# TrevorS/qwen3-tts-rs

Measured on AMD Instinct MI355X. Metric: acoustic_frames_per_sec, higher is better.
Workload: dtype bf16

## Files before the change

qwen3_tts_rs_amd/csrc/q3_codec_stream.hip:

```cpp
#include "q3_engine.h"

struct CsRow { int pos = 0; float* kv = nullptr; float* lat = nullptr; float* hist = nullptr; std::vector<float*> blocks; };
struct q3_codec_stream {
    q3_model* m = nullptr; int R = 0, cap = 0;
    int bf = 0, max_blocks = 0;
    std::vector<float*> free_blocks; int blocks_total = 0, blocks_in_use = 0, blocks_peak = 0;
    hipStream_t st = nullptr; bool owns_stream = false;
    std::vector<CsRow> rows;
    CodecWS ws;
    float *cs = nullptr, *sn = nullptr;
    char* desc = nullptr; size_t desc_cap = 0;
    float* stage = nullptr; float* stage_host = nullptr; size_t stage_cap = 0;
};

static size_t kv_floats(const q3_codec_stream* cs) {
    const q3_config& c = cs->m->cfg;
    return (size_t)c.dec_layers * 2 * c.dec_heads * c.dec_head_dim * cs->cap;
}

static size_t block_floats(const q3_codec_stream* cs) {
    const q3_config& c = cs->m->cfg;
    return ((size_t)c.dec_layers * 2 * c.dec_heads * c.dec_head_dim + c.dec_latent) * cs->bf;
}

q3_status codec_stream_create(q3_model* m, int rows, int max_frames, hipStream_t st, q3_codec_stream** out, int block_frames, int max_blocks) {
    if (!m || !m->finalized) return set_err(Q3_INVALID_ARG, "model not finalized");
    if (!out || rows < 1 || max_frames < 1) return set_err(Q3_INVALID_ARG, "q3_codec_stream_create: rows and max_frames must be positive");
    if (m->device < 0) return set_err(Q3_INVALID_ARG, "q3_codec_stream_create: the model has no device (manifest-only): the vocoder runs on the GPU");
    if (m->cfg.dec_head_dim != 64) return set_err(Q3_INVALID_ARG, "q3_codec_stream_create: decoder head dim must be 64");
    HIPC(hipSetDevice(m->device));
    std::unique_ptr<q3_codec_stream> cs(new q3_codec_stream());
    cs->m = m; cs->R = rows; cs->cap = max_frames; cs->rows.resize(rows);
    cs->bf = block_frames; cs->max_blocks = max_blocks;
    m->refs.fetch_add(1);
    auto fail = [&](q3_status s) { q3_codec_stream_free(cs.release()); return s; };
// ... 22 lines not shown
    if (max_blocks < 0) return set_err(Q3_INVALID_ARG, "q3_codec_stream_create_blocked: negative max_blocks");
    return codec_stream_create(m, rows, max_frames, nullptr, out, block_frames, max_blocks);
}
extern "C" q3_status q3_codec_stream_info(q3_codec_stream* cs, int* block_frames, size_t* block_bytes, int* blocks_total, int* blocks_in_use, int* blocks_peak) {
    if (!cs) return set_err(Q3_INVALID_ARG, "q3_codec_stream_info: null stream");
    if (block_frames) *block_frames = cs->bf;
    if (block_bytes) *block_bytes = block_floats(cs) * 4;
    if (blocks_total) *blocks_total = cs->blocks_total;
    if (blocks_in_use) *blocks_in_use = cs->blocks_in_use;
    if (blocks_peak) *blocks_peak = cs->blocks_peak;
    return Q3_OK;
}

extern "C" void q3_codec_stream_free(q3_codec_stream* cs) {
    if (!cs) return;
    q3_model* m = cs->m;
    (void)hipSetDevice(m->device);
    if (cs->st) (void)hipStreamSynchronize(cs->st);
    for (CsRow& r : cs->rows) { dev_free(r.kv); dev_free(r.lat); dev_free(r.hist); for (float* b : r.blocks) dev_free(b); }
    for (float* b : cs->free_blocks) dev_free(b);
    cs->ws.release();
    dev_free(cs->cs); dev_free(cs->sn); dev_free(cs->desc); dev_free(cs->stage);
    if (cs->stage_host) (void)hipHostFree(cs->stage_host);
    if (cs->owns_stream && cs->st) (void)hipStreamDestroy(cs->st);
    delete cs;
    if (m->refs.fetch_sub(1) == 1) model_destroy(m);
}

int codec_stream_pos(const q3_codec_stream* cs, int row) { return cs->rows[row].pos; }
void codec_stream_blocks(const q3_codec_stream* cs, int row, int upto, int* held, int* need) {
    const CsRow& r = cs->rows[row];
    *held = (int)r.blocks.size();
    *need = cs->bf ? std::max(0, (upto + cs->bf - 1) / cs->bf - *held) : 0;
}
void codec_stream_reset(q3_codec_stream* cs, int row) {
    CsRow& r = cs->rows[row];
    r.pos = 0;
    cs->blocks_in_use -= (int)r.blocks.size();
    cs->free_blocks.insert(cs->free_blocks.end(), r.blocks.begin(), r.blocks.end());
    r.blocks.clear();
}

extern "C" q3_status q3_codec_stream_reset(q3_codec_stream* cs, int row) {
    if (!cs || row < 0 || row >= cs->R) return set_err(Q3_INVALID_ARG, "q3_codec_stream_reset: bad row");
    codec_stream_reset(cs, row);
    return Q3_OK;
}
extern "C" q3_status q3_codec_stream_pos(q3_codec_stream* cs, int row, int* n_frames) {
    if (!cs || row < 0 || row >= cs->R || !n_frames) return set_err(Q3_INVALID_ARG, "q3_codec_stream_pos: bad row");
    *n_frames = cs->rows[row].pos;
    return Q3_OK;
}

namespace {
struct DescBlock {
    std::vector<char> host;
    template <typename T> size_t add(const std::vector<T>& v) {
        const size_t off = (host.size() + 15) & ~(size_t)15;
        host.resize(off + v.size() * sizeof(T));
        if (!v.empty()) memcpy(host.data() + off, v.data(), v.size() * sizeof(T));
        return off;
    }
};
}

q3_status codec_stream_push(q3_codec_stream* cs, const std::vector<CsPush>& all) {
    q3_model* m = cs->m;
    const q3_config& c = m->cfg;
    std::vector<CsPush> P;
    for (const CsPush& p : all) if (p.n > 0) P.push_back(p);
    q3_pcm_stage* ps = nullptr;
    std::vector<const CsPush*> flush;
    for (const CsPush& p : all) {
        if (p.ps) ps = p.ps;
        if (p.n_out) *p.n_out = 0;
        if (p.n <= 0 && p.ps && p.last) flush.push_back(&p);
    }
    if (P.empty()) {
        if (flush.empty()) return Q3_OK;
        std::vector<PsSeg> segs; std::vector<void*> outs; std::vector<size_t> cnt(flush.size(), 0);
        for (const CsPush* f : flush) { segs.push_back({f->ps_row, nullptr, 0, 1}); outs.push_back(f->out_host); }
        Q3C(pcm_stage_push_dev(ps, segs, cs->st, outs.data(), cnt.data()));
        for (size_t k = 0; k < flush.size(); ++k) if (flush[k]->n_out) *flush[k]->n_out = cnt[k];
        return Q3_OK;
    }
    HIPC(hipSetDevice(m->device));
    hipStream_t st = cs->st;
    const int Q = c.dec_q_dim, LAT = c.dec_latent, QD = c.dec_heads * c.dec_head_dim, cap = cs->cap, spf = samples_per_frame(c);
    const int nP = (int)P.size();
// ... 43 lines not shown
        CsRow& r = cs->rows[p.row];
        if (bf || r.kv) continue;
        if (dev_malloc((void**)&r.kv, kv_floats(cs) * 4) != hipSuccess || dev_malloc((void**)&r.lat, (size_t)LAT * cap * 4) != hipSuccess ||
            dev_malloc((void**)&r.hist, (size_t)Q * 2 * 4) != hipSuccess) {
            (void)hipGetLastError();
            dev_free(r.kv); dev_free(r.lat); dev_free(r.hist); r.kv = r.lat = r.hist = nullptr;
            return set_err(Q3_OOM, "codec stream: state of row %d (%zu MB)", p.row, (kv_floats(cs) + (size_t)LAT * cap) * 4 >> 20);
        }
    }
    int N = 0, W = 0, Lc = 0, solo_max = 0, max_tiles = 0;
    std::vector<int> col0(nP), out0(nP), conc, solo;
    for (int i = 0; i < nP; ++i) {
        const int f0 = cs->rows[P[i].row].pos, a0 = f0 + P[i].skip, e = f0 + P[i].n;
        col0[i] = N; N += P[i].n;
        out0[i] = W; W += e - a0;
        if (e > a0) {
            if (a0 > CODEC_CTX_FRAMES) { conc.push_back(i); Lc += e - a0 + CODEC_CTX_FRAMES; }
            else { solo.push_back(i); solo_max = std::max(solo_max, e); }
        }
        max_tiles = std::max(max_tiles, ((e - 1) >> 5) - (f0 >> 5) + 1);
    }
    const int Np = N + 2 * nP;
    {
        const int CS_WIDE = 2048;
        int max_n = 0; for (const CsPush& p : P) max_n = std::max(max_n, p.n);
        const int T = std::max(1, std::max(Lc, solo_max));
        const long long Tw = (long long)cs->R * (max_n + CODEC_CTX_FRAMES), Fw = (long long)cs->R * (max_n + 2);
        Q3C(codec_reserve(m, cs->ws, (int)std::max<long long>(T, std::min<long long>(Tw, CS_WIDE)),
                          (int)std::max<long long>(Np, std::min<long long>(Fw, CS_WIDE))));
    }
    CodecWS& ws = cs->ws;
    if ((size_t)W * spf > cs->stage_cap) {
        HIPC(hipStreamSynchronize(st));
        dev_free(cs->stage); cs->stage = nullptr;
        if (cs->stage_host) { (void)hipHostFree(cs->stage_host); cs->stage_host = nullptr; }
        cs->stage_cap = 0;
        HIPC(dev_malloc((void**)&cs->stage, (size_t)W * spf * 4));
        HIPC(hipHostMalloc((void**)&cs->stage_host, (size_t)W * spf * 4, hipHostMallocDefault));
        cs->stage_cap = (size_t)W * spf;
    }
    std::vector<PsSeg> psegs; std::vector<const CsPush*> pseg_of; std::vector<void*> pouts; PsPlan plan;
    if (ps) {
        for (int i = 0; i < nP; ++i)
            if (P[i].ps) { psegs.push_back({P[i].ps_row, cs->stage + (size_t)out0[i] * spf, (size_t)(P[i].n - P[i].skip) * spf, P[i].last}); pseg_of.push_back(&P[i]); }
        for (const CsPush* f : flush) { psegs.push_back({f->ps_row, nullptr, 0, 1}); pseg_of.push_back(f); }
        for (const CsPush* p : pseg_of) pouts.push_back(p->out_host);
        Q3C(pcm_stage_begin(ps, psegs, plan));
    }
    float *A = ws.bufA, *B = ws.bufB, *C = ws.bufC, *F = ws.bufF;
    float* knew = A + (size_t)QD * N;
    std::vector<int> pos(N);
    std::vector<AttnCsRow> arows(nP);
    std::vector<ColCopy> xin(Np), hist(2 * nP), compact(N), kvsc(N), latsc(N), latg(Lc), solog;
    std::vector<SegCopy> segs;
    std::vector<AttnCbRow> brows(bf ? nP : 0);
    std::vector<const float*> tabs;
    auto kv_col = [&](const CsRow& r, int f) { return bf ? r.blocks[f / bf] + f % bf : r.kv + f; };
    auto lat_col = [&](const CsRow& r, int f) { return bf ? r.blocks[f / bf] + lat_off + f % bf : r.lat + f; };
    std::vector<const uint32_t*> fsrc(on_dev ? N : 0);
    std::vector<uint32_t> fhost(on_dev ? 0 : (size_t)N * 16);
    for (int i = 0; i < nP; ++i) {
        const CsRow& r = cs->rows[P[i].row];
// ... 13 lines not shown
            else memcpy(&fhost[(size_t)col * 16], P[i].host + (size_t)j * 16, 64);
        }
    }
    {
        int l0 = 0;
        for (int i : conc) {
            const CsRow& r = cs->rows[P[i].row];
            const int a0 = r.pos + P[i].skip, c0 = a0 - CODEC_CTX_FRAMES, len = P[i].n - P[i].skip + CODEC_CTX_FRAMES;
            for (int j = 0; j < len; ++j) latg[l0 + j] = {lat_col(r, c0 + j), F + l0 + j, kp, Lc};
            segs.push_back({(unsigned long long)(l0 + CODEC_CTX_FRAMES) * spf, (unsigned long long)out0[i] * spf, (unsigned long long)(P[i].n - P[i].skip) * spf});
            l0 += len;
        }
        for (int i : solo) {
            const CsRow& r = cs->rows[P[i].row];
            const int e = r.pos + P[i].n;
            if (bf) for (int f = 0; f < e; ++f) solog.push_back({lat_col(r, f), F + f, kp, e});
            segs.push_back({(unsigned long long)(cs->rows[P[i].row].pos + P[i].skip) * spf, (unsigned long long)out0[i] * spf,
                            (unsigned long long)(P[i].n - P[i].skip) * spf});
        }
    }
    DescBlock db;
    const size_t o_pos = db.add(pos), o_arows = db.add(arows), o_xin = db.add(xin), o_hist = db.add(hist), o_compact = db.add(compact),
                 o_kvsc = db.add(kvsc), o_latsc = db.add(latsc), o_latg = db.add(latg), o_segs = db.add(segs), o_fsrc = db.add(fsrc),
                 o_brows = db.add(brows), o_tabs = db.add(tabs), o_solog = db.add(solog), o_ps = db.add(plan.desc);
    if (db.host.size() > cs->desc_cap) {
        HIPC(hipStreamSynchronize(st));
        dev_free(cs->desc); cs->desc = nullptr; cs->desc_cap = 0;
        HIPC(dev_malloc((void**)&cs->desc, db.host.size() * 2));
        cs->desc_cap = db.host.size() * 2;
    }
    struct Failed {
        q3_codec_stream* cs; const std::vector<CsPush>& P; bool armed = true;
        ~Failed() {
            if (!armed) return;
            (void)hipStreamSynchronize(cs->st);
            for (const CsPush& p : P) codec_stream_reset(cs, p.row);
        }
    } failed{cs, P};
    HIPC(q3_hipMemcpy(cs->desc, db.host.data(), db.host.size(), hipMemcpyHostToDevice));
    auto D = [&](size_t off) { return (const void*)(cs->desc + off); };
    if (on_dev) HIPC(launch_gather_frames((const uint32_t* const*)D(o_fsrc), ws.frames, N, st));
    else HIPC(q3_hipMemcpy(ws.frames, fhost.data(), fhost.size() * 4, hipMemcpyHostToDevice));

    const CodecScope scope(m);
    Q3C(codec_front_quant(m, ws, N, st));
    HIPC(launch_copy_cols((const ColCopy*)D(o_xin), Np, Q, 0, 0, st));
    HIPC(launch_copy_cols((const ColCopy*)D(o_hist), 2 * nP, Q, 0, 0, st));
    Q3C(codec_front_preconv(m, A, B, Np, st));
    HIPC(launch_copy_cols((const ColCopy*)D(o_compact), N, LAT, 0, 0, st));
    const float scale = (float)pow((double)c.dec_head_dim, -0.5);
    Q3C(codec_front_transformer(m, ws, N, st, [&](int l, float* q, float* k, float*, float* ao) -> q3_status {
        const size_t layer_off = (size_t)l * 2 * QD * kp;
        HIPC(launch_rope_c_pos(q, k, cs->cs, cs->sn, (const int*)D(o_pos), c.dec_heads, c.dec_head_dim, N, st));
        HIPC(launch_copy_cols((const ColCopy*)D(o_kvsc), N, 2 * QD, 0, layer_off, st));
        if (bf) HIPC(launch_attn_cb(q, ao, (const AttnCbRow*)D(o_brows), (const float* const*)D(o_tabs), nP, max_tiles, layer_off, c.dec_heads, c.dec_head_dim, N, bf, scale, st));
        else HIPC(launch_attn_cs(q, ao, (const AttnCsRow*)D(o_arows), nP, max_tiles, layer_off, c.dec_heads, c.dec_head_dim, N, cap, scale, st));
        return Q3_OK;
    }));
    HIPC(launch_copy_cols((const ColCopy*)D(o_latsc), N, LAT, 0, 0, st));
    const SegCopy* dsegs = (const SegCopy*)D(o_segs);
    if (!conc.empty()) {
        size_t max_n = 0; for (int i : conc) max_n = std::max(max_n, (size_t)(P[i].n - P[i].skip) * spf);
        HIPC(launch_copy_cols((const ColCopy*)D(o_latg), Lc, LAT, 0, 0, st));
        Q3C(codec_stack_dev(m, ws, F, Lc, st, nullptr, scope));
        HIPC(launch_copy_segs(ws.pcm, cs->stage, dsegs, (int)conc.size(), max_n, st));
    }
    for (size_t k = 0, g0 = 0; k < solo.size(); ++k) {
        const int i = solo[k]; const CsRow& r = cs->rows[P[i].row];
        const int e = r.pos + P[i].n;
        if (bf) { HIPC(launch_copy_cols((const ColCopy*)D(o_solog) + g0, e, LAT, 0, 0, st)); g0 += (size_t)e; }
        else HIPC(launch_copy_rows(r.lat, cap, F, e, LAT, e, st));
        Q3C(codec_stack_dev(m, ws, F, e, st, nullptr, scope));
        HIPC(launch_copy_segs(ws.pcm, cs->stage, dsegs + conc.size() + k, 1, (size_t)(P[i].n - P[i].skip) * spf, st));
    }
    bool raw = false;
    for (int i = 0; i < nP; ++i) raw = raw || !P[i].ps;
    if (W > 0 && raw) HIPC(hipMemcpyAsync(cs->stage_host, cs->stage, (size_t)W * spf * 4, hipMemcpyDeviceToHost, st));
    if (ps) Q3C(pcm_stage_run(ps, psegs, plan, (const PsDesc*)D(o_ps), st));
    HIPC(hipStreamSynchronize(st));
    if (ps) pcm_stage_finish(ps, psegs, plan, pouts.data(), nullptr);
    for (size_t k = 0; k < psegs.size(); ++k) if (pseg_of[k]->n_out) *pseg_of[k]->n_out = plan.count[k];
    for (int i = 0; i < nP; ++i) {
        if (P[i].pcm_host && !P[i].ps) memcpy(P[i].pcm_host, cs->stage_host + (size_t)out0[i] * spf, (size_t)(P[i].n - P[i].skip) * spf * 4);
        cs->rows[P[i].row].pos += P[i].n;
    }
    failed.armed = false; untake.armed = false;
    cs->blocks_peak = std::max(cs->blocks_peak, cs->blocks_in_use);
    return Q3_OK;
}

extern "C" q3_status q3_codec_stream_push(q3_codec_stream* cs, int n_rows, const int* rows, const uint32_t* const* frames_host,
                                          const int* n_frames, float* const* pcm_host, const size_t* cap) {
    if (!cs) return set_err(Q3_INVALID_ARG, "q3_codec_stream_push: null stream");
    if (n_rows < 0 || (n_rows > 0 && (!rows || !frames_host || !n_frames || !pcm_host || !cap)))
        return set_err(Q3_INVALID_ARG, "q3_codec_stream_push: null argument");
    const int spf = samples_per_frame(cs->m->cfg);
    std::vector<char> seen(cs->R, 0);
    std::vector<CsPush> P;
    for (int i = 0; i < n_rows; ++i) {
        const int r = rows[i], n = n_frames[i];
        if (r < 0 || r >= cs->R) return set_err(Q3_INVALID_ARG, "q3_codec_stream_push: row %d out of range (%d rows)", r, cs->R);
        if (seen[r]) return set_err(Q3_INVALID_ARG, "q3_codec_stream_push: row %d listed twice", r);
        seen[r] = 1;
        if (n < 0) return set_err(Q3_INVALID_ARG, "q3_codec_stream_push: negative frame count for row %d", r);
        if (n == 0) continue;
        if (cs->rows[r].pos + n > cs->cap)
// ... 61 lines not shown
```

qwen3_tts_rs_amd/csrc/q3_engine.h:

```cpp
#pragma once
#include "../../include/q3tts.h"
#include "q3_kernels.h"

#include <math.h>
#include <stdarg.h>
#include <stdio.h>
#include <string.h>

#include <algorithm>
#include <atomic>
#include <chrono>
#include <functional>
#include <memory>
#include <string>
#include <thread>
#include <mutex>
#include <unordered_map>
#include <vector>

#include "q3_internal.h"
#include "q3_aql.h"

using namespace q3;
#define Q3_HIDDEN __attribute__((visibility("hidden")))
// ... 317 lines not shown
    bool kv_bf16 = false, kv_in_bf16 = false; unsigned long long* kv_conv = nullptr;
    float *rows = nullptr, *embeds = nullptr, *xvec = nullptr; int n_rows_total = 0;
    uint32_t* ids_dev = nullptr; int *tr_dev = nullptr, *ci_dev = nullptr; float *proj_e = nullptr, *proj_h = nullptr;
    uint32_t* ref_codes_dev = nullptr;
    int *trail_base = nullptr, *trail_len = nullptr, *pad_row = nullptr;
    int* text_ready = nullptr;
    uint32_t* app_ids = nullptr; float *app_e = nullptr, *app_h = nullptr, *app_out = nullptr;
    int* flush_buf = nullptr; size_t flush_cap = 0;
    uint32_t* tok = nullptr; uint8_t* seen = nullptr; int *frame_idx = nullptr, *pos = nullptr, *token_count = nullptr;
    float* U = nullptr; uint32_t* codes = nullptr;
    float* logits_hist = nullptr; float* cp_logits_hist = nullptr; bool debug = false;
    bool prefilled = false; int frames_run = 0;
    uint64_t uid = 0; char* park_desc = nullptr; std::shared_ptr<ParkShelf> shelf;
    hipGraphExec_t graph_exec = nullptr; hipGraph_t graph = nullptr;
    q3::AqlProgram* aql = nullptr; int aql_mode = 0; bool aql_tried = false, aql_failed = false;
    bool precapture = false;
    CodecWS cws;
    q3_codec_stream* cstream = nullptr;
    q3_pcm_stage* ostage = nullptr; bool out_started = false;
    std::vector<OutSettings> out;
    hipStream_t dec_stream = nullptr; hipEvent_t dec_ev = nullptr;
    std::vector<CodecWS> par_ws; std::vector<hipStream_t> par_streams;
    CodecWS seg_ws;
    std::vector<uint32_t> codes_host; bool codes_host_valid = false;
    int stream_mode = 0;
    bool profile = false; ProfAcc prof_linear;
    bool legacy_attn = getenv("Q3_LEGACY_ATTN") != nullptr;
    bool proj_tables = getenv("Q3_NO_PROJ_TABLES") == nullptr;
    bool qkv_tables = getenv("Q3_NO_QKV_TABLES") == nullptr;
    bool ksplit = getenv("Q3_NO_KSPLIT") == nullptr;
    bool cp_attn = getenv("Q3_NO_CP_ATTN") == nullptr;
    bool no_chunk = getenv("Q3_NO_CHUNK") != nullptr;
    std::vector<std::pair<hipEvent_t, hipEvent_t>> prof_events; std::vector<double> prof_event_bytes;
    std::vector<hipEvent_t> prof_pool; size_t prof_pool_next = 0;
    std::vector<ProfShape> prof_shapes;
#ifdef Q3_TRACE
    unsigned long long* trace_buf = nullptr; int trace_node = 0, trace_cap = 0;
    struct TraceMeta { int kind, a, b, c, d, e, f; };
    std::vector<TraceMeta> trace_meta;
    unsigned long long* trace_next(int kind, int a, int b, int c, int d = 0, int e = 0, int f = 0) {
        if (!trace_buf || trace_node >= trace_cap) return nullptr;
        trace_meta.push_back({kind, a, b, c, d, e, f});
        return trace_buf + (size_t)(trace_node++) * TRACE_NODE;
    }
#endif
    ~q3_session();
// ... 1 lines not shown


Q3_HIDDEN void model_destroy(q3_model* m);
Q3_HIDDEN void retile_bf16(const uint16_t* src, int N, int K, uint16_t* dst, int mode);
Q3_HIDDEN q3_status codec_reserve(const q3_model* m, CodecWS& ws, int T, int Tf = 0);
Q3_HIDDEN int samples_per_frame(const q3_config& c);
Q3_HIDDEN q3_status codec_decode_dev(const q3_model* m, CodecWS& ws, int T, hipStream_t st, float** taps, int c0 = 0, int resident = 0);
struct VocodeSrc { const uint32_t* prefix_host; int n_prefix;
                   const uint32_t* codes; bool codes_on_host; };
struct VocodePcm { const float* dev; size_t n; };
Q3_HIDDEN int vocode_ctx_start(int a);
Q3_HIDDEN q3_status vocode_enqueue(const q3_model* m, CodecWS& ws, hipStream_t st, const VocodeSrc& src, int a, int e, int c0, int resident, VocodePcm* out);
Q3_HIDDEN q3_status vocode_copy_out(const VocodePcm& pcm, float* host, size_t cap, size_t* n, hipStream_t st);
struct Q3_HIDDEN CodecScope { int planes, resident; explicit CodecScope(const q3_model* m, int resident = 0); ~CodecScope(); CodecScope(const CodecScope&) = delete; };
using CodecAttnFn = std::function<q3_status(int layer, float* q, float* k, float* v, float* ao)>;
Q3_HIDDEN q3_status codec_rope_table(const q3_config& c, int n, float* cs_dev, float* sn_dev);
Q3_HIDDEN q3_status codec_front_quant(const q3_model* m, CodecWS& ws, int T, hipStream_t st);
Q3_HIDDEN q3_status codec_front_preconv(const q3_model* m, const float* x, float* y, int L, hipStream_t st);
Q3_HIDDEN q3_status codec_front_transformer(const q3_model* m, CodecWS& ws, int T, hipStream_t st, const CodecAttnFn& rope_attn);
Q3_HIDDEN q3_status codec_stack_dev(const q3_model* m, CodecWS& ws, float* cur, int L, hipStream_t st, float** taps, const CodecScope& scope);
struct CsPush {
    int row; int n; int skip; const uint32_t* host; const uint32_t* dev; float* pcm_host;
    q3_pcm_stage* ps = nullptr; int ps_row = -1; int last = 0; void* out_host = nullptr; size_t* n_out = nullptr;
};
Q3_HIDDEN q3_status codec_stream_create(q3_model* m, int rows, int max_frames, hipStream_t st, q3_codec_stream** out, int block_frames = 0,
                                        int max_blocks = 0);
Q3_HIDDEN q3_status codec_stream_push(q3_codec_stream* cs, const std::vector<CsPush>& pushes);
Q3_HIDDEN int codec_stream_pos(const q3_codec_stream* cs, int row);
Q3_HIDDEN void codec_stream_blocks(const q3_codec_stream* cs, int row, int upto, int* held, int* need);
Q3_HIDDEN void codec_stream_reset(q3_codec_stream* cs, int row);
struct PsSeg { int row; const float* dev; size_t n; int last; };
struct PsDesc {
    const float* src; const float* tail_in; float* tail_out; const float* taps; void* out;
    long long base, i0;
    int n_new, n_out, L, M, fmt, pad;
};
struct PsPlan { std::vector<PsDesc> desc; std::vector<size_t> off, count; size_t bytes = 0; bool late = false; };
Q3_HIDDEN void resampler_taps(int L, int M, std::vector<float>& out);
Q3_HIDDEN uint64_t synth_hash(uint64_t x);
Q3_HIDDEN uint64_t synth_name_hash(const char* s);
Q3_HIDDEN void mark_carrier(uint64_t key, float* c);
Q3_HIDDEN q3_status mark_score_f32(const float* rho, double* score, int* offset);
Q3_HIDDEN int pcm_stage_rows(const q3_pcm_stage* ps);
Q3_HIDDEN void pcm_stage_reset(q3_pcm_stage* ps, int row);
Q3_HIDDEN q3_status pcm_stage_check_rows(const q3_pcm_stage* ps, const char* who, int n_rows, const int* rows);
Q3_HIDDEN size_t pcm_stage_count(const q3_pcm_stage* ps, int row, size_t n, int last);
Q3_HIDDEN q3_status out_set_output(const char* who, OutSettings& o, uint32_t sample_rate, int format);
Q3_HIDDEN q3_status out_set_tempo(const char* who, OutSettings& o, int tempo_permille);
Q3_HIDDEN q3_status out_set_pitch(const char* who, OutSettings& o, int cents);
Q3_HIDDEN q3_status out_set_level(const char* who, OutSettings& o, int gain_mB, int ceiling_mB);
// ... 51 lines not shown
```

qwen3_tts_rs_amd/csrc/q3_session.hip:

```cpp
#include "q3_engine.h"
#include "q3_prefix_cache.h"

hipError_t sync_frames(q3_session* s) {
    if (s->aql) {
        std::string why;
        if (!q3::aql_wait(s->aql, &why)) { s->aql_failed = true; set_err(Q3_HIP_ERROR, "AQL frame submission: %s", why.c_str()); return hipErrorUnknown; }
    }
    return hipStreamSynchronize(s->stream);
}

static hipError_t run_linear(q3_session* s, const LinArgs& a_in) {
    LinArgs a = a_in;
    a.ws = s->wide_ws; a.ws_bytes = s->wide_ws_bytes;
#ifdef Q3_TRACE
    a.trace = s->trace_next(0, a.M, a.N, a.K, a.epi, a.norm_w ? 1 : 0, a.tiled);
#endif
    if (!s->profile) return launch_linear(a, s->stream);
    hipEvent_t e0, e1;
    if (s->prof_pool_next + 2 <= s->prof_pool.size()) { e0 = s->prof_pool[s->prof_pool_next++]; e1 = s->prof_pool[s->prof_pool_next++]; }
    else {
        hipError_t e = hipEventCreate(&e0); if (e != hipSuccess) return e;
        e = hipEventCreate(&e1); if (e != hipSuccess) return e;
        s->prof_pool.push_back(e0); s->prof_pool.push_back(e1); s->prof_pool_next = s->prof_pool.size();
    }
// ... 591 lines not shown
    return Q3_OK;
}

q3_session::~q3_session() {
    if (!m) return;
    (void)hipSetDevice(m->device);
    if (stream) (void)hipStreamSynchronize(stream);
    if (dec_stream) (void)hipStreamSynchronize(dec_stream);
    for (auto st : par_streams) (void)hipStreamSynchronize(st);
    if (aql) q3::aql_program_destroy(aql);
    for (int b = 0; b < (int)kv_rows.size(); ++b) kv_release_row(this, b);
    if (shelf) {
        std::lock_guard<std::mutex> g(shelf->mu);
        shelf->alive = false;
        for (auto& blk : shelf->blocks) dev_free(blk.first);
        shelf->blocks.clear();
    }
    if (graph_exec) (void)hipGraphExecDestroy(graph_exec);
    if (graph) (void)hipGraphDestroy(graph);
    for (auto& ev : prof_pool) (void)hipEventDestroy(ev);
    for (auto st : par_streams) (void)hipStreamDestroy(st);
    if (ostage) q3_pcm_stage_free(ostage);
    if (cstream) q3_codec_stream_free(cstream);
    cws.release(); seg_ws.release();
    for (auto& w : par_ws) w.release();
    if (dec_ev) (void)hipEventDestroy(dec_ev);
    if (dec_stream) (void)hipStreamDestroy(dec_stream);
    if (stream && owns_stream) {
        std::lock_guard<std::mutex> g(m->stream_mu);
        if (m->idle_streams.size() < 16) { m->idle_streams.push_back(stream); stream = nullptr; }
    }
    if (stream && owns_stream) (void)hipStreamDestroy(stream);
    pool.release_all();
    if (m->refs.fetch_sub(1) == 1) model_destroy(m);
}

extern "C" void q3_session_free(q3_session* s) { delete s; }

extern "C" q3_status q3_session_set_kv_dtype(q3_session* s, int dtype) {
    if (!s) return set_err(Q3_INVALID_ARG, "null session");
    if (s->prefilled) return set_err(Q3_INVALID_ARG, "q3_session_set_kv_dtype must be called before prefill");
    if (dtype != Q3_DTYPE_F32 && dtype != Q3_DTYPE_BF16) return set_err(Q3_INVALID_ARG, "q3_session_set_kv_dtype: unknown dtype %d", dtype);
    if (dtype == Q3_DTYPE_BF16 && !s->paged) return set_err(Q3_UNSUPPORTED, "bf16 K/V needs the paged cache (Q3_KV_CONTIGUOUS is set)");
    s->kv_bf16 = dtype == Q3_DTYPE_BF16;
    return Q3_OK;
}
// ... 1195 lines not shown

extern "C" q3_status q3_session_decode(q3_session* s, int b, int f0, int f1, float* pcm_host, size_t cap, size_t* n_samples) {
    if (!s || b < 0 || b >= s->B) return set_err(Q3_INVALID_ARG, "bad sequence index");
    HIPC(hipSetDevice(s->m->device));
    Q3C(refresh_codes(s));
    if (f0 < 0 || f1 < f0 || f1 > s->seq[b].n_frames) return set_err(Q3_INVALID_ARG, "bad frame range [%d,%d) of %d", f0, f1, s->seq[b].n_frames);
    if (n_samples) *n_samples = 0;
    if (f1 == f0) return Q3_OK;
    VocodePcm pcm;
    Q3C(vocode_enqueue(s->m, s->cws, s->stream, row_src(s, b, f0, f0 == 0 && f1 == s->seq[b].n_frames), 0, f1 - f0, 0, 0, &pcm));
    HIPC(sync_frames(s));
    return vocode_copy_out(pcm, pcm_host, cap, n_samples, nullptr);
}

using run_clk = std::chrono::steady_clock;
static double run_ms(run_clk::time_point a, run_clk::time_point b) { return std::chrono::duration<double, std::milli>(b - a).count(); }
struct RunKnobs {
    int overlap;
    int resident;
    int seg, tail;
    int pairs;
    int cus;
    bool log;
};
static int env_int(const char* name, int unset) { const char* e = getenv(name); return e ? atoi(e) : unset; }
static RunKnobs read_run_knobs() {
    static const int pairs = std::min(std::max(env_int("Q3_DECODE_PAIRS", 2), 1), 8);
    static const int cus = [] { const int v = env_int("Q3_DECODE_CUS", 0); return v <= 0 ? 0 : (v < 8 ? 8 : (v > 248 ? 248 : v & ~7)); }();
    const char* overlap = getenv("Q3_DECODE_OVERLAP");
    return {overlap ? (atoi(overlap) != 0 ? 1 : 0) : -1, std::min(std::max(env_int("Q3_DECODE_RESIDENT", 1), 0), 2),
            std::max(env_int("Q3_DECODE_SEG", 256), 16), std::max(env_int("Q3_DECODE_TAIL", 32), 16), pairs, cus, getenv("Q3_DECODE_LOG") != nullptr};
}
struct Lane { CodecWS& ws; hipStream_t st; };
static q3_status decode_lanes(q3_session* s, int n) {
    while ((int)s->par_ws.size() < n - 1) {
        hipStream_t st = nullptr;
        HIPC(hipStreamCreateWithFlags(&st, hipStreamNonBlocking));
        s->par_ws.emplace_back(); s->par_streams.push_back(st);
    }
    return Q3_OK;
}
static Lane lane(q3_session* s, int k) { return k == 0 ? Lane{s->cws, s->stream} : Lane{s->par_ws[(size_t)k - 1], s->par_streams[(size_t)k - 1]}; }

static q3_status run_serial(q3_session* s, int use_graph, const RunKnobs& kn, float** pcm_host, const size_t* cap, run_clk::time_point* frames_done) {
    Q3C(q3_session_generate(s, s->max_frames, use_graph));
    Q3C(refresh_codes(s));
    *frames_done = run_clk::now();
    const int spf = samples_per_frame(s->m->cfg), conc = kn.pairs;
    bool any_icl = false;
    for (auto& q : s->seq) any_icl = any_icl || !q.ref_codes.empty();
    if (conc == 1 || s->B == 1 || any_icl) {
        for (int b = 0; b < s->B; ++b) Q3C(q3_session_decode(s, b, 0, s->seq[b].n_frames, pcm_host ? pcm_host[b] : nullptr, cap ? cap[b] : 0, nullptr));
        return Q3_OK;
    }
// ... 17 lines not shown
}

static constexpr bool DECODE_OVERLAP_DEFAULT = true;
struct SegJob { int b, a, e; };
static q3_status seg_enqueue(q3_session* s, const SegJob& j, CodecWS& ws, hipStream_t st, int resident, float** pcm_host, const size_t* cap) {
    const size_t at = (size_t)j.a * samples_per_frame(s->m->cfg);
    float* host = pcm_host ? pcm_host[j.b] : nullptr;
    VocodePcm pcm;
    Q3C(vocode_enqueue(s->m, ws, st, row_src(s, j.b), j.a, j.e, vocode_ctx_start(j.a), resident, &pcm));
    return vocode_copy_out(pcm, host ? host + at : nullptr, cap && cap[j.b] > at ? cap[j.b] - at : 0, nullptr, st);
}
static std::vector<SegJob> seg_collect(const q3_session* s, std::vector<int>& dec_pos, int seg, bool final_pass) {
    std::vector<SegJob> jobs;
    for (int b = 0; b < s->B; ++b) {
        const SeqInfo& q = s->seq[b];
        const int e = (q.done || final_pass) ? q.n_frames : (q.n_frames < s->frames_run ? q.n_frames : s->frames_run);
        if (e > dec_pos[(size_t)b] && (final_pass || q.done || e - dec_pos[(size_t)b] >= 16)) {
            for (int a = dec_pos[(size_t)b]; a < e; a += seg) jobs.push_back({b, a, a + seg < e ? a + seg : e});
            dec_pos[(size_t)b] = e;
        }
    }
    return jobs;
}
struct OverlapMarks { run_clk::time_point frames_done; int n_dispatch = 0; double join_wait_ms = 0.0; };
static q3_status run_overlapped(q3_session* s, int use_graph, const RunKnobs& kn, float** pcm_host, const size_t* cap, OverlapMarks* marks) {
    HIPC(hipSetDevice(s->m->device));
    if (!s->dec_stream) {
        if (kn.cus) {
            uint32_t mask[8] = {0, 0, 0, 0, 0, 0, 0, 0};
            for (int i = 256 - kn.cus; i < 256; ++i) mask[i >> 5] |= 1u << (i & 31);
            HIPC(hipExtStreamCreateWithCUMask(&s->dec_stream, 8, mask));
        } else {
            int least = 0, greatest = 0;
            HIPC(hipDeviceGetStreamPriorityRange(&least, &greatest));
            HIPC(hipStreamCreateWithPriority(&s->dec_stream, hipStreamNonBlocking, least));
        }
    }
    Q3C(codec_reserve(s->m, s->seg_ws, kn.seg + CODEC_CTX_FRAMES, s->max_frames));
    struct Split {
        q3::AqlProgram* p = nullptr;
        void release() { if (p) { std::string why; q3::aql_restrict_cus(p, 0, &why); p = nullptr; } }
        ~Split() { release(); }
    } split;
    if (kn.cus && s->aql && !s->aql_failed) { std::string why; if (q3::aql_restrict_cus(s->aql, 256 - kn.cus, &why)) split.p = s->aql; }
    std::vector<int> dec_pos((size_t)s->B, 0);
    std::thread worker; q3_status wst = Q3_OK; std::string werr;
    auto join = [&]() -> q3_status {
        if (worker.joinable()) worker.join();
        if (wst != Q3_OK) return set_err(wst, "%s", werr.c_str());
        return Q3_OK;
    };
    auto dispatch = [&]() -> q3_status {
        std::vector<SegJob> jobs = seg_collect(s, dec_pos, kn.seg, false);
        if (jobs.empty()) return Q3_OK;
        {
            const auto j0 = run_clk::now();
            Q3C(join());
            marks->join_wait_ms += run_ms(j0, run_clk::now()); ++marks->n_dispatch;
        }
        worker = std::thread([s, jobs, resident = kn.resident, pcm_host, cap, &wst, &werr]() {
            if (hipSetDevice(s->m->device) != hipSuccess) { wst = Q3_HIP_ERROR; werr = "hipSetDevice failed in the decode thread"; return; }
            for (const SegJob& j : jobs) {
                const q3_status st = seg_enqueue(s, j, s->seg_ws, s->dec_stream, resident, pcm_host, cap);
                if (st != Q3_OK) { wst = st; werr = q3_last_error(); return; }
            }
        });
        return Q3_OK;
    };
    q3_status st = Q3_OK;
    while (st == Q3_OK && session_remaining(s) > 0 && !all_done(s)) {
        int n = kn.seg;
        const int left = session_remaining(s);
        if (left > kn.tail && left - n < kn.tail) n = left - kn.tail;
        st = q3_session_generate(s, n, use_graph);
        if (st == Q3_OK) st = refresh_codes(s);
        if (st == Q3_OK && session_remaining(s) > 0 && !all_done(s)) st = dispatch();
    }
    marks->frames_done = run_clk::now();
    split.release();
    { const q3_status js = join(); if (st == Q3_OK) st = js; }
    if (st != Q3_OK) { hipStreamSynchronize(s->dec_stream); return st; }
    const int conc = 2;
    auto tail = [&]() -> q3_status {
        std::vector<SegJob> jobs = seg_collect(s, dec_pos, kn.seg, true);
        Q3C(decode_lanes(s, conc));
        for (int k = 0; k < conc; ++k) Q3C(codec_reserve(s->m, lane(s, k).ws, kn.seg + CODEC_CTX_FRAMES, s->max_frames));
        for (size_t i = 0; i < jobs.size(); ++i) { const Lane ln = lane(s, (int)(i % conc)); Q3C(seg_enqueue(s, jobs[i], ln.ws, ln.st, 0, pcm_host, cap)); }
        return Q3_OK;
    };
    st = tail();
    hipError_t he = hipStreamSynchronize(s->dec_stream);
    for (int k = 0; k < conc && k <= (int)s->par_streams.size(); ++k) { const hipError_t e2 = hipStreamSynchronize(lane(s, k).st); if (he == hipSuccess) he = e2; }
    if (st != Q3_OK) return st;
    HIPC(he);
    return Q3_OK;
}

extern "C" q3_status q3_session_run(q3_session* s, int use_graph, float** pcm_host, const size_t* cap, size_t* n_samples, q3_timing* timing) {
    if (!s) return set_err(Q3_INVALID_ARG, "null session");
    if (any_open_text(s)) return set_err(Q3_UNSUPPORTED, "q3_session_run: a row's text is still open (q3_session_append_text with last != 0 closes it; or drive the session with q3_session_generate)");
    const auto t0 = run_clk::now();
    s->precapture = use_graph != 0;
    Q3C(q3_session_prefill(s));
    const auto t1 = run_clk::now();
    const RunKnobs kn = read_run_knobs();
    const bool overlap_wanted = kn.overlap >= 0 ? kn.overlap != 0 : (DECODE_OVERLAP_DEFAULT && s->B >= 2 && s->B <= 16);
    bool overlap = overlap_wanted && !s->debug && !s->profile && s->max_frames > kn.seg;
    for (auto& q : s->seq) if (!q.ref_codes.empty()) overlap = false;
    OverlapMarks marks;
    Q3C(overlap ? run_overlapped(s, use_graph, kn, pcm_host, cap, &marks) : run_serial(s, use_graph, kn, pcm_host, cap, &marks.frames_done));
    int total = 0;
    for (int b = 0; b < s->B; ++b) {
        if (n_samples) n_samples[b] = (size_t)s->seq[b].n_frames * samples_per_frame(s->m->cfg);
        total += s->seq[b].n_frames;
    }
    const auto t2 = marks.frames_done, t3 = run_clk::now();
    if (timing) { timing->prefill_ms = run_ms(t0, t1); timing->generation_ms = run_ms(t1, t2); timing->decode_ms = run_ms(t2, t3); timing->generation_frames = total; }
    if (overlap && kn.log)
        fprintf(stderr, "q3_session_run overlap: resident %d seg %d tail %d, %d dispatches, frame loop waited %.3f ms for the enqueue thread, frames %.1f ms, exposed decode %.1f ms\n",
                kn.resident, kn.seg, kn.tail, marks.n_dispatch, marks.join_wait_ms, run_ms(t1, t2), run_ms(t2, t3));
    return Q3_OK;
}

extern "C" q3_status q3_session_set_stream_mode(q3_session* s, int mode) {
    if (!s || (mode != 0 && mode != 1)) return set_err(Q3_INVALID_ARG, "q3_session_set_stream_mode: mode must be 0 (context-free) or 1 (continuous)");
    s->stream_mode = mode;
    return Q3_OK;
}

extern "C" q3_status q3_session_next_chunk(q3_session* s, float* pcm_host, size_t cap, size_t* n_samples, int* done) {
    if (!s) return set_err(Q3_INVALID_ARG, "null session");
    if (s->B != 1) return set_err(Q3_UNSUPPORTED, "streaming sessions are batch 1 (StreamingSession, lib.rs:1484)");
    if (!s->prefilled) { s->precapture = true; Q3C(q3_session_prefill(s)); }
    Q3C(refresh_codes(s));
    Q3C(chunk_fill(s, 0));
    const ChunkCut cut = chunk_cut(s, 0);
    if (cut.avail <= 0) { if (n_samples) *n_samples = 0; if (done) *done = cut.ends ? 1 : 0; return Q3_OK; }
    SeqInfo& q = s->seq[0];
    const int chunk = chunk_frames_of(s), avail = cut.avail;
    static const bool no_ahead = getenv("Q3_STREAM_NO_AHEAD") != nullptr;
    int ahead = 0;
    if (!no_ahead && !q.done && (s->aql || s->graph_exec) && !s->aql_failed && !s->debug && !s->profile) {
        ahead = chunk - (q.n_frames - (q.stream_pos + avail));
// ... 72 lines not shown
```

Before: 2885.

## Decode overlapped segments through a stateful codec stream with grouped async pushes

```diff
diff --git a/qwen3_tts_rs_amd/csrc/q3_codec_stream.hip b/qwen3_tts_rs_amd/csrc/q3_codec_stream.hip
--- a/qwen3_tts_rs_amd/csrc/q3_codec_stream.hip
+++ b/qwen3_tts_rs_amd/csrc/q3_codec_stream.hip
@@ -10,7 +10,9 @@
     CodecWS ws;
     float *cs = nullptr, *sn = nullptr;
     char* desc = nullptr; size_t desc_cap = 0;
-    float* stage = nullptr; float* stage_host = nullptr; size_t stage_cap = 0;
+    char* desc_host = nullptr; size_t desc_host_cap = 0;
+    float* stage = nullptr; size_t stage_cap = 0;
+    float* stage_host = nullptr; size_t stage_host_cap = 0;
 };
 
 static size_t kv_floats(const q3_codec_stream* cs) {
@@ -79,6 +81,7 @@
     cs->ws.release();
     dev_free(cs->cs); dev_free(cs->sn); dev_free(cs->desc); dev_free(cs->stage);
     if (cs->stage_host) (void)hipHostFree(cs->stage_host);
+    if (cs->desc_host) (void)hipHostFree(cs->desc_host);
     if (cs->owns_stream && cs->st) (void)hipStreamDestroy(cs->st);
     delete cs;
     if (m->refs.fetch_sub(1) == 1) model_destroy(m);
@@ -106,6 +109,69 @@
 extern "C" q3_status q3_codec_stream_pos(q3_codec_stream* cs, int row, int* n_frames) {
     if (!cs || row < 0 || row >= cs->R || !n_frames) return set_err(Q3_INVALID_ARG, "q3_codec_stream_pos: bad row");
     *n_frames = cs->rows[row].pos;
+    return Q3_OK;
+}
+
+static q3_status grow_stage(q3_codec_stream* cs, size_t samples, bool host) {
+    if (samples > cs->stage_cap) {
+        dev_free(cs->stage); cs->stage = nullptr; cs->stage_cap = 0;
+        HIPC(dev_malloc((void**)&cs->stage, samples * 4));
+        cs->stage_cap = samples;
+    }
+    if (host && samples > cs->stage_host_cap) {
+        if (cs->stage_host) { (void)hipHostFree(cs->stage_host); cs->stage_host = nullptr; }
+        cs->stage_host_cap = 0;
+        HIPC(hipHostMalloc((void**)&cs->stage_host, samples * 4, hipHostMallocDefault));
+        cs->stage_host_cap = samples;
+    }
+    return Q3_OK;
+}
+static q3_status grow_desc(q3_codec_stream* cs, size_t bytes, bool host) {
+    if (bytes > cs->desc_cap) {
+        dev_free(cs->desc); cs->desc = nullptr; cs->desc_cap = 0;
+        HIPC(dev_malloc((void**)&cs->desc, bytes));
+        cs->desc_cap = bytes;
+    }
+    if (host && bytes > cs->desc_host_cap) {
+        if (cs->desc_host) { (void)hipHostFree(cs->desc_host); cs->desc_host = nullptr; }
+        cs->desc_host_cap = 0;
+        HIPC(hipHostMalloc((void**)&cs->desc_host, bytes, hipHostMallocDefault));
+        cs->desc_host_cap = bytes;
+    }
+    return Q3_OK;
+}
+static q3_status reserve_ws(q3_codec_stream* cs, int cols, int front, int max_n) {
+    const int CS_WIDE = 2048;
+    const long long Tw = (long long)cs->R * (max_n + CODEC_CTX_FRAMES), Fw = (long long)cs->R * (max_n + 2);
+    return codec_reserve(cs->m, cs->ws, (int)std::max<long long>(std::max(1, cols), std::min<long long>(Tw, CS_WIDE)),
+                         (int)std::max<long long>(front, std::min<long long>(Fw, CS_WIDE)));
+}
+
+q3_status codec_stream_presize(q3_codec_stream* cs, int rows, int frames, int max_n, int cols) {
+    q3_model* m = cs->m;
+    const q3_config& c = m->cfg;
+    HIPC(hipSetDevice(m->device));
+    HIPC(hipStreamSynchronize(cs->st));
+    rows = std::min(rows, cs->R); frames = std::min(frames, cs->cap);
+    cols = std::max(cols, max_n + CODEC_CTX_FRAMES);
+    Q3C(reserve_ws(cs, cols, cols, max_n));
+    Q3C(grow_stage(cs, (size_t)cols * samples_per_frame(c), false));
+    const size_t per_row_blocks = cs->bf ? (size_t)(cs->cap + cs->bf - 1) / cs->bf : 0;
+    Q3C(grow_desc(cs, (size_t)cols * (4 + 8 + 64 + 7 * sizeof(ColCopy)) +
+                          (size_t)rows * (sizeof(AttnCsRow) + sizeof(AttnCbRow) + sizeof(SegCopy) + 4 * sizeof(ColCopy) + per_row_blocks * 8) + 16 * 16, true));
+    for (int r = 0; r < rows; ++r) {
+        CsRow& row = cs->rows[(size_t)r];
+        if (cs->bf && !row.hist && dev_malloc((void**)&row.hist, (size_t)c.dec_q_dim * 2 * 4) != hipSuccess) { (void)hipGetLastError(); row.hist = nullptr; break; }
+    }
+    if (cs->bf) {
+        long long want = (long long)rows * ((frames + cs->bf - 1) / cs->bf);
+        if (cs->max_blocks > 0) want = std::min<long long>(want, cs->max_blocks);
+        while (cs->blocks_total < want) {
+            float* b = nullptr;
+            if (dev_malloc((void**)&b, block_floats(cs) * 4) != hipSuccess) { (void)hipGetLastError(); break; }
+            cs->free_blocks.push_back(b); cs->blocks_total++;
+        }
+    }
     return Q3_OK;
 }
 
@@ -121,7 +187,7 @@
 };
 }
 
-q3_status codec_stream_push(q3_codec_stream* cs, const std::vector<CsPush>& all) {
+q3_status codec_stream_push(q3_codec_stream* cs, const std::vector<CsPush>& all, const CsPushOpts& opts) {
     q3_model* m = cs->m;
     const q3_config& c = m->cfg;
     std::vector<CsPush> P;
@@ -211,22 +277,15 @@
     }
     const int Np = N + 2 * nP;
     {
-        const int CS_WIDE = 2048;
         int max_n = 0; for (const CsPush& p : P) max_n = std::max(max_n, p.n);
-        const int T = std::max(1, std::max(Lc, solo_max));
-        const long long Tw = (long long)cs->R * (max_n + CODEC_CTX_FRAMES), Fw = (long long)cs->R * (max_n + 2);
-        Q3C(codec_reserve(m, cs->ws, (int)std::max<long long>(T, std::min<long long>(Tw, CS_WIDE)),
-                          (int)std::max<long long>(Np, std::min<long long>(Fw, CS_WIDE))));
+        Q3C(reserve_ws(cs, std::max(Lc, solo_max), Np, max_n));
     }
     CodecWS& ws = cs->ws;
-    if ((size_t)W * spf > cs->stage_cap) {
+    bool bounce = false;
+    for (int i = 0; i < nP; ++i) bounce = bounce || (!P[i].ps && !P[i].direct);
+    if ((size_t)W * spf > cs->stage_cap || (bounce && (size_t)W * spf > cs->stage_host_cap)) {
         HIPC(hipStreamSynchronize(st));
-        dev_free(cs->stage); cs->stage = nullptr;
-        if (cs->stage_host) { (void)hipHostFree(cs->stage_host); cs->stage_host = nullptr; }
-        cs->stage_cap = 0;
-        HIPC(dev_malloc((void**)&cs->stage, (size_t)W * spf * 4));
-        HIPC(hipHostMalloc((void**)&cs->stage_host, (size_t)W * spf * 4, hipHostMallocDefault));
-        cs->stage_cap = (size_t)W * spf;
+        Q3C(grow_stage(cs, (size_t)W * spf, bounce));
     }
     std::vector<PsSeg> psegs; std::vector<const CsPush*> pseg_of; std::vector<void*> pouts; PsPlan plan;
     if (ps) {
@@ -286,12 +345,11 @@
     DescBlock db;
     const size_t o_pos = db.add(pos), o_arows = db.add(arows), o_xin = db.add(xin), o_hist = db.add(hist), o_compact = db.add(compact),
                  o_kvsc = db.add(kvsc), o_latsc = db.add(latsc), o_latg = db.add(latg), o_segs = db.add(segs), o_fsrc = db.add(fsrc),
-                 o_brows = db.add(brows), o_tabs = db.add(tabs), o_solog = db.add(solog), o_ps = db.add(plan.desc);
-    if (db.host.size() > cs->desc_cap) {
+                 o_brows = db.add(brows), o_tabs = db.add(tabs), o_solog = db.add(solog), o_ps = db.add(plan.desc),
+                 o_fhost = opts.async ? db.add(fhost) : 0;
+    if (db.host.size() > cs->desc_cap || (opts.async && db.host.size() > cs->desc_host_cap)) {
         HIPC(hipStreamSynchronize(st));
-        dev_free(cs->desc); cs->desc = nullptr; cs->desc_cap = 0;
-        HIPC(dev_malloc((void**)&cs->desc, db.host.size() * 2));
-        cs->desc_cap = db.host.size() * 2;
+        Q3C(grow_desc(cs, db.host.size() * 2, opts.async));
     }
     struct Failed {
         q3_codec_stream* cs; const std::vector<CsPush>& P; bool armed = true;
@@ -301,12 +359,16 @@
             for (const CsPush& p : P) codec_stream_reset(cs, p.row);
         }
     } failed{cs, P};
-    HIPC(q3_hipMemcpy(cs->desc, db.host.data(), db.host.size(), hipMemcpyHostToDevice));
+    if (opts.async) {
+        memcpy(cs->desc_host, db.host.data(), db.host.size());
+        HIPC(hipMemcpyAsync(cs->desc, cs->desc_host, db.host.size(), hipMemcpyHostToDevice, st));
+    } else HIPC(q3_hipMemcpy(cs->desc, db.host.data(), db.host.size(), hipMemcpyHostToDevice));
     auto D = [&](size_t off) { return (const void*)(cs->desc + off); };
     if (on_dev) HIPC(launch_gather_frames((const uint32_t* const*)D(o_fsrc), ws.frames, N, st));
+    else if (opts.async) HIPC(hipMemcpyAsync(ws.frames, D(o_fhost), fhost.size() * 4, hipMemcpyDeviceToDevice, st));
     else HIPC(q3_hipMemcpy(ws.frames, fhost.data(), fhost.size() * 4, hipMemcpyHostToDevice));
 
-    const CodecScope scope(m);
+    const CodecScope scope(m, opts.resident);
     Q3C(codec_front_quant(m, ws, N, st));
     HIPC(launch_copy_cols((const ColCopy*)D(o_xin), Np, Q, 0, 0, st));
     HIPC(launch_copy_cols((const ColCopy*)D(o_hist), 2 * nP, Q, 0, 0, st));
@@ -337,15 +399,16 @@
         Q3C(codec_stack_dev(m, ws, F, e, st, nullptr, scope));
         HIPC(launch_copy_segs(ws.pcm, cs->stage, dsegs + conc.size() + k, 1, (size_t)(P[i].n - P[i].skip) * spf, st));
     }
-    bool raw = false;
-    for (int i = 0; i < nP; ++i) raw = raw || !P[i].ps;
-    if (W > 0 && raw) HIPC(hipMemcpyAsync(cs->stage_host, cs->stage, (size_t)W * spf * 4, hipMemcpyDeviceToHost, st));
+    if (W > 0 && bounce) HIPC(hipMemcpyAsync(cs->stage_host, cs->stage, (size_t)W * spf * 4, hipMemcpyDeviceToHost, st));
+    for (int i = 0; i < nP; ++i)
+        if (P[i].direct && !P[i].ps && P[i].pcm_host && P[i].n > P[i].skip)
+            HIPC(hipMemcpyAsync(P[i].pcm_host, cs->stage + (size_t)out0[i] * spf, (size_t)(P[i].n - P[i].skip) * spf * 4, hipMemcpyDeviceToHost, st));
     if (ps) Q3C(pcm_stage_run(ps, psegs, plan, (const PsDesc*)D(o_ps), st));
     HIPC(hipStreamSynchronize(st));
     if (ps) pcm_stage_finish(ps, psegs, plan, pouts.data(), nullptr);
     for (size_t k = 0; k < psegs.size(); ++k) if (pseg_of[k]->n_out) *pseg_of[k]->n_out = plan.count[k];
     for (int i = 0; i < nP; ++i) {
-        if (P[i].pcm_host && !P[i].ps) memcpy(P[i].pcm_host, cs->stage_host + (size_t)out0[i] * spf, (size_t)(P[i].n - P[i].skip) * spf * 4);
+        if (P[i].pcm_host && !P[i].ps && !P[i].direct) memcpy(P[i].pcm_host, cs->stage_host + (size_t)out0[i] * spf, (size_t)(P[i].n - P[i].skip) * spf * 4);
         cs->rows[P[i].row].pos += P[i].n;
     }
     failed.armed = false; untake.armed = false;
diff --git a/qwen3_tts_rs_amd/csrc/q3_engine.h b/qwen3_tts_rs_amd/csrc/q3_engine.h
--- a/qwen3_tts_rs_amd/csrc/q3_engine.h
+++ b/qwen3_tts_rs_amd/csrc/q3_engine.h
@@ -363,6 +363,7 @@
     hipStream_t dec_stream = nullptr; hipEvent_t dec_ev = nullptr;
     std::vector<CodecWS> par_ws; std::vector<hipStream_t> par_streams;
     CodecWS seg_ws;
+    q3_codec_stream* dstream = nullptr; int dstream_bf = 0, dstream_blocks = 0;
     std::vector<uint32_t> codes_host; bool codes_host_valid = false;
     int stream_mode = 0;
     bool profile = false; ProfAcc prof_linear;
@@ -410,10 +411,13 @@
 struct CsPush {
     int row; int n; int skip; const uint32_t* host; const uint32_t* dev; float* pcm_host;
     q3_pcm_stage* ps = nullptr; int ps_row = -1; int last = 0; void* out_host = nullptr; size_t* n_out = nullptr;
-};
+    int direct = 0;
+};
+struct CsPushOpts { int resident = 0; bool async = false; };
 Q3_HIDDEN q3_status codec_stream_create(q3_model* m, int rows, int max_frames, hipStream_t st, q3_codec_stream** out, int block_frames = 0,
                                         int max_blocks = 0);
-Q3_HIDDEN q3_status codec_stream_push(q3_codec_stream* cs, const std::vector<CsPush>& pushes);
+Q3_HIDDEN q3_status codec_stream_push(q3_codec_stream* cs, const std::vector<CsPush>& pushes, const CsPushOpts& opts = CsPushOpts());
+Q3_HIDDEN q3_status codec_stream_presize(q3_codec_stream* cs, int rows, int frames, int max_n, int cols);
 Q3_HIDDEN int codec_stream_pos(const q3_codec_stream* cs, int row);
 Q3_HIDDEN void codec_stream_blocks(const q3_codec_stream* cs, int row, int upto, int* held, int* need);
 Q3_HIDDEN void codec_stream_reset(q3_codec_stream* cs, int row);
diff --git a/qwen3_tts_rs_amd/csrc/q3_session.hip b/qwen3_tts_rs_amd/csrc/q3_session.hip
--- a/qwen3_tts_rs_amd/csrc/q3_session.hip
+++ b/qwen3_tts_rs_amd/csrc/q3_session.hip
@@ -637,6 +637,7 @@
     for (auto st : par_streams) (void)hipStreamDestroy(st);
     if (ostage) q3_pcm_stage_free(ostage);
     if (cstream) q3_codec_stream_free(cstream);
+    if (dstream) q3_codec_stream_free(dstream);
     cws.release(); seg_ws.release();
     for (auto& w : par_ws) w.release();
     if (dec_ev) (void)hipEventDestroy(dec_ev);
@@ -1878,14 +1879,21 @@
     int pairs;
     int cus;
     bool log;
+    int state;
+    int group;
+    int state_blocks;
+    int state_bf;
 };
 static int env_int(const char* name, int unset) { const char* e = getenv(name); return e ? atoi(e) : unset; }
+static constexpr int DECODE_STATE_DEFAULT = 1;
 static RunKnobs read_run_knobs() {
     static const int pairs = std::min(std::max(env_int("Q3_DECODE_PAIRS", 2), 1), 8);
     static const int cus = [] { const int v = env_int("Q3_DECODE_CUS", 0); return v <= 0 ? 0 : (v < 8 ? 8 : (v > 248 ? 248 : v & ~7)); }();
     const char* overlap = getenv("Q3_DECODE_OVERLAP");
     return {overlap ? (atoi(overlap) != 0 ? 1 : 0) : -1, std::min(std::max(env_int("Q3_DECODE_RESIDENT", 1), 0), 2),
-            std::max(env_int("Q3_DECODE_SEG", 256), 16), std::max(env_int("Q3_DECODE_TAIL", 32), 16), pairs, cus, getenv("Q3_DECODE_LOG") != nullptr};
+            std::max(env_int("Q3_DECODE_SEG", 256), 16), std::max(env_int("Q3_DECODE_TAIL", 32), 16), pairs, cus, getenv("Q3_DECODE_LOG") != nullptr,
+            env_int("Q3_DECODE_STATE", DECODE_STATE_DEFAULT) != 0 ? 1 : 0, std::max(env_int("Q3_DECODE_GROUP", 2048), 1), std::max(env_int("Q3_DECODE_STATE_BLOCKS", 0), 0),
+            std::max(env_int("Q3_DECODE_STATE_BLOCK", 128), 32) / 32 * 32};
 }
 struct Lane { CodecWS& ws; hipStream_t st; };
 static q3_status decode_lanes(q3_session* s, int n) {
@@ -1949,7 +1957,36 @@
     }
     return jobs;
 }
-struct OverlapMarks { run_clk::time_point frames_done; int n_dispatch = 0; double join_wait_ms = 0.0; };
+struct StateRun { bool on = false, fell_back = false; int pushes = 0, groups = 0; };
+static q3_status state_push(q3_session* s, const std::vector<SegJob>& jobs, const RunKnobs& kn, int resident, float** pcm_host, const size_t* cap, StateRun& sr) {
+    const size_t spf = (size_t)samples_per_frame(s->m->cfg);
+    for (const SegJob& j : jobs)
+        if (pcm_host && pcm_host[j.b] && (!cap || cap[j.b] < (size_t)j.e * spf)) return set_err(Q3_INVALID_ARG, "pcm buffer too small");
+    for (size_t i = 0; i < jobs.size();) {
+        if (sr.on && !sr.fell_back) {
+            std::vector<CsPush> P; int cols = 0; size_t k = i;
+            for (; k < jobs.size(); ++k) {
+                const SegJob& j = jobs[k];
+                bool twice = false; for (const CsPush& p : P) twice = twice || p.row == j.b;
+                if (!P.empty() && (twice || cols + j.e - j.a + CODEC_CTX_FRAMES > kn.group)) break;
+                if (codec_stream_pos(s->dstream, j.b) != j.a) return set_err(Q3_INVALID_ARG, "q3_session_run: the decode stream has row %d at frame %d, its segment starts at %d", j.b, codec_stream_pos(s->dstream, j.b), j.a);
+                CsPush p{j.b, j.e - j.a, 0, nullptr, s->codes + ((size_t)j.b * s->max_frames + j.a) * 16, pcm_host ? pcm_host[j.b] : nullptr};
+                if (p.pcm_host) p.pcm_host += (size_t)j.a * spf;
+                p.direct = 1;
+                P.push_back(p); cols += j.e - j.a + CODEC_CTX_FRAMES;
+            }
+            CsPushOpts o; o.resident = resident; o.async = true;
+            const q3_status st = codec_stream_push(s->dstream, P, o);
+            if (st == Q3_OK) { sr.pushes += (int)P.size(); sr.groups++; i = k; continue; }
+            if (st != Q3_OOM) return st;
+            sr.fell_back = true;
+        }
+        Q3C(seg_enqueue(s, jobs[i], s->seg_ws, s->dec_stream, resident, pcm_host, cap));
+        ++i;
+    }
+    return Q3_OK;
+}
+struct OverlapMarks { run_clk::time_point frames_done; int n_dispatch = 0; double join_wait_ms = 0.0, tail_wait_ms = 0.0; StateRun state; };
 static q3_status run_overlapped(q3_session* s, int use_graph, const RunKnobs& kn, float** pcm_host, const size_t* cap, OverlapMarks* marks) {
     HIPC(hipSetDevice(s->m->device));
     if (!s->dec_stream) {
@@ -1964,6 +2001,21 @@
         }
     }
     Q3C(codec_reserve(s->m, s->seg_ws, kn.seg + CODEC_CTX_FRAMES, s->max_frames));
+    StateRun& sr = marks->state;
+    sr.on = kn.state != 0;
+    if (sr.on) {
+        if (s->dstream && (s->dstream_bf != kn.state_bf || s->dstream_blocks != kn.state_blocks)) { q3_codec_stream_free(s->dstream); s->dstream = nullptr; }
+        q3_status cst = Q3_OK;
+        if (!s->dstream) {
+            cst = codec_stream_create(s->m, s->B, s->max_frames, s->dec_stream, &s->dstream, kn.state_bf, kn.state_blocks);
+            if (cst == Q3_OK) { s->dstream_bf = kn.state_bf; s->dstream_blocks = kn.state_blocks; } else s->dstream = nullptr;
+        }
+        if (cst == Q3_OK) {
+            for (int b = 0; b < s->B; ++b) codec_stream_reset(s->dstream, b);
+            cst = codec_stream_presize(s->dstream, s->B, s->max_frames, kn.seg, std::min(kn.group, s->B * (kn.seg + CODEC_CTX_FRAMES)));
+        }
+        if (cst == Q3_OOM) sr.fell_back = true; else Q3C(cst);
+    }
     struct Split {
         q3::AqlProgram* p = nullptr;
         void release() { if (p) { std::string why; q3::aql_restrict_cus(p, 0, &why); p = nullptr; } }
@@ -1985,10 +2037,15 @@
             Q3C(join());
             marks->join_wait_ms += run_ms(j0, run_clk::now()); ++marks->n_dispatch;
         }
-        worker = std::thread([s, jobs, resident = kn.resident, pcm_host, cap, &wst, &werr]() {
+        worker = std::thread([s, jobs, kn, pcm_host, cap, &sr, &wst, &werr]() {
             if (hipSetDevice(s->m->device) != hipSuccess) { wst = Q3_HIP_ERROR; werr = "hipSetDevice failed in the decode thread"; return; }
+            if (sr.on) {
+                const q3_status st = state_push(s, jobs, kn, kn.resident, pcm_host, cap, sr);
+                if (st != Q3_OK) { wst = st; werr = q3_last_error(); }
+                return;
+            }
             for (const SegJob& j : jobs) {
-                const q3_status st = seg_enqueue(s, j, s->seg_ws, s->dec_stream, resident, pcm_host, cap);
+                const q3_status st = seg_enqueue(s, j, s->seg_ws, s->dec_stream, kn.resident, pcm_host, cap);
                 if (st != Q3_OK) { wst = st; werr = q3_last_error(); return; }
             }
         });
@@ -2006,10 +2063,12 @@
     marks->frames_done = run_clk::now();
     split.release();
     { const q3_status js = join(); if (st == Q3_OK) st = js; }
+    marks->tail_wait_ms = run_ms(marks->frames_done, run_clk::now());
     if (st != Q3_OK) { hipStreamSynchronize(s->dec_stream); return st; }
     const int conc = 2;
     auto tail = [&]() -> q3_status {
         std::vector<SegJob> jobs = seg_collect(s, dec_pos, kn.seg, true);
+        if (sr.on && !sr.fell_back) return state_push(s, jobs, kn, 0, pcm_host, cap, sr);
         Q3C(decode_lanes(s, conc));
         for (int k = 0; k < conc; ++k) Q3C(codec_reserve(s->m, lane(s, k).ws, kn.seg + CODEC_CTX_FRAMES, s->max_frames));
         for (size_t i = 0; i < jobs.size(); ++i) { const Lane ln = lane(s, (int)(i % conc)); Q3C(seg_enqueue(s, jobs[i], ln.ws, ln.st, 0, pcm_host, cap)); }
@@ -2044,8 +2103,10 @@
     const auto t2 = marks.frames_done, t3 = run_clk::now();
     if (timing) { timing->prefill_ms = run_ms(t0, t1); timing->generation_ms = run_ms(t1, t2); timing->decode_ms = run_ms(t2, t3); timing->generation_frames = total; }
     if (overlap && kn.log)
-        fprintf(stderr, "q3_session_run overlap: resident %d seg %d tail %d, %d dispatches, frame loop waited %.3f ms for the enqueue thread, frames %.1f ms, exposed decode %.1f ms\n",
-                kn.resident, kn.seg, kn.tail, marks.n_dispatch, marks.join_wait_ms, run_ms(t1, t2), run_ms(t2, t3));
+        fprintf(stderr, "q3_session_run overlap: resident %d seg %d tail %d, %d dispatches, frame loop waited %.3f ms for the enqueue thread, frames %.1f ms, exposed decode %.1f ms"
+                        ", state %s, %d pushes in %d groups (at most %d columns), tail waited %.1f ms for the segments in flight\n",
+                kn.resident, kn.seg, kn.tail, marks.n_dispatch, marks.join_wait_ms, run_ms(t1, t2), run_ms(t2, t3),
+                !marks.state.on ? "off" : (marks.state.fell_back ? "fell back" : "on"), marks.state.pushes, marks.state.groups, kn.group, marks.tail_wait_ms);
     return Q3_OK;
 }
 
```

Result: no change. 2906, median of 6 (+0.7%).
